# angeladai/sgnn

Hardware: AMD Instinct MI355X
Metric: TSDF blocks/sec fwd+bwd (64^3@5% occ, bs32) (higher is better)
Workload: dtype f32

## Files before the change

sgnn_amd/csrc/bn.hip:

```cpp
#include "common.h"

#define BN_MAX_BLOCKS 2048
#define BN_FLUSH 2
#ifndef BN_U
#define BN_U 2
#endif
#define BN_FUSE_BLOCKS 4096
#define BN_FUSE_MAXC 64

struct BnGeom {
  int vec;
  int cq;
  int rpb;
};

static BnGeom bn_geom(int c) {
  BnGeom g;
  g.vec = (c % 4 == 0) ? 4 : 1;
  g.cq = c / g.vec;
  g.rpb = 256 / g.cq;
  if (g.rpb < 1) g.rpb = 1;
  return g;
}

// ... 6 lines not shown
  return g;
}

static int bn_blocks(int64_t n, const BnGeom &g) {
  int64_t b = (n + (int64_t)g.rpb * BN_FLUSH - 1) / ((int64_t)g.rpb * BN_FLUSH);
  if (b < 1) b = 1;
  if (b > BN_MAX_BLOCKS) b = BN_MAX_BLOCKS;
  return (int)b;
}

SGNN_EXPORT int64_t sgnn_bn_ws_bytes(int64_t n, int c) {
  (void)n;
  return (int64_t)BN_MAX_BLOCKS * 2 * c * (int64_t)sizeof(double) + 4 * (int64_t)c * sizeof(float) + 256;
}

template <int VEC>
__device__ __forceinline__ void load_vec(const float *p, float (&v)[VEC]) {
  if constexpr (VEC == 4) {
    const float4 t = *reinterpret_cast<const float4 *>(p);
    v[0] = t.x; v[1] = t.y; v[2] = t.z; v[3] = t.w;
  } else {
    v[0] = *p;
  }
}
template <int VEC>
__device__ __forceinline__ void store_vec(float *p, const float (&v)[VEC]) {
  if constexpr (VEC == 4) {
    *reinterpret_cast<float4 *>(p) = make_float4(v[0], v[1], v[2], v[3]);
  } else {
    *p = v[0];
  }
}

template <int VEC, int MODE, bool LIN = false>
__global__ __launch_bounds__(256) void k_bn_partial(const float *__restrict__ x, int64_t ldx,
                                                   const float *__restrict__ dy, int64_t ld_dy, int64_t n, int c,
                                                   int cq, int rpb, const float *__restrict__ mean,
                                                   const float *__restrict__ invstd,
                                                   const float *__restrict__ gamma,
                                                   const float *__restrict__ beta, float leak,
                                                   double *__restrict__ partial, const int64_t *n_dev, BnLin lin) {
  extern __shared__ double sh[];
  const int tid = threadIdx.x;
  unsigned nblk = gridDim.x;
  if (n_dev) {
    n = sgnn_dyn_n(n, n_dev);
    int64_t b = (n + (int64_t)rpb * BN_FLUSH - 1) / ((int64_t)rpb * BN_FLUSH);
    if (b < 1) b = 1;
    if (b > BN_MAX_BLOCKS) b = BN_MAX_BLOCKS;
    if (b < (int64_t)nblk) nblk = (unsigned)b;
    if (blockIdx.x >= nblk) {
      for (int o = tid; o < 2 * c; o += 256) partial[(size_t)blockIdx.x * 2 * c + o] = 0.0;
      return;
    }
  }
  const int col = tid % cq, rloc = tid / cq;
  const bool active = rloc < rpb;
  double sa[VEC], sb[VEC];
#pragma unroll
  for (int v = 0; v < VEC; ++v) sa[v] = sb[v] = 0.0;
  float m_[VEC], is_[VEC], g_[VEC], b_[VEC];
  float lw[2][VEC];
  if constexpr (LIN) {
#pragma unroll
    for (int o = 0; o < 2; ++o)
#pragma unroll
      for (int v = 0; v < VEC; ++v) lw[o][v] = (active && o < lin.nout) ? lin.w[o][col * VEC + v] : 0.f;
  }
  if (MODE == 1 && active) {
#pragma unroll
    for (int v = 0; v < VEC; ++v) {
      m_[v] = mean[col * VEC + v];
      is_[v] = invstd[col * VEC + v];
      g_[v] = gamma ? gamma[col * VEC + v] : 1.f;
      b_[v] = beta ? beta[col * VEC + v] : 0.f;
    }
  }
  if (active) {
    const int64_t step = (int64_t)nblk * rpb;
    int64_t row = (int64_t)blockIdx.x * rpb + rloc;
    while (row < n) {
      float fa[VEC], fb[VEC];
#pragma unroll
      for (int v = 0; v < VEC; ++v) fa[v] = fb[v] = 0.f;
      float xv[BN_FLUSH][VEC], dv[BN_FLUSH][VEC];
      bool keep[BN_FLUSH];
#pragma unroll
      for (int it = 0; it < BN_FLUSH; ++it) {
        const int64_t rr = row + it * step;
        keep[it] = rr < n;
        const int64_t rc = rr < n ? rr : row;
        load_vec<VEC>(x + rc * ldx + col * VEC, xv[it]);
        if constexpr (LIN) {
#pragma unroll
          for (int v = 0; v < VEC; ++v) dv[it][v] = 0.f;
#pragma unroll
          for (int o = 0; o < 2; ++o)
            if (o < lin.nout) {
              const float gv = lin.g[rc * lin.ldg + o];
#pragma unroll
              for (int v = 0; v < VEC; ++v) dv[it][v] = fmaf(gv, lw[o][v], dv[it][v]);
            }
        } else if (MODE == 1) {
          load_vec<VEC>(dy + rc * ld_dy + col * VEC, dv[it]);
        }
      }
#pragma unroll
      for (int it = 0; it < BN_FLUSH; ++it) {
        if (MODE == 0) {
#pragma unroll
          for (int v = 0; v < VEC; ++v) {
            const float xm = keep[it] ? xv[it][v] : 0.f;
            fa[v] += xm;
            fb[v] = fmaf(xm, xm, fb[v]);
          }
        } else {
#pragma unroll
          for (int v = 0; v < VEC; ++v) {
            const float xh = (xv[it][v] - m_[v]) * is_[v];
            const float yv = fmaf(xh, g_[v], b_[v]);
            const float dz = keep[it] ? (yv > 0.f ? dv[it][v] : dv[it][v] * leak) : 0.f;
            fa[v] += dz;
            fb[v] = fmaf(dz, xh, fb[v]);
          }
        }
      }
      row += (int64_t)BN_FLUSH * step;
#pragma unroll
      for (int v = 0; v < VEC; ++v) {
        sa[v] += (double)fa[v];
        sb[v] += (double)fb[v];
      }
    }
  }
  double *mine = sh + ((size_t)rloc * cq + col) * 2 * VEC;
// ... 422 lines not shown
                               float leak, float *save_mean, float *save_invstd, float *y, int64_t ldy,
                               const double *pre_partial, int64_t pre_nblk, void *ws, int64_t ws_bytes,
                               sgnn_stream_t stream) {
  return sgnn_bn_fwd_impl(x, ldx, n, c, gamma, beta, running_mean, running_var, eps, momentum, training, leak,
                          save_mean, save_invstd, y, ldy, pre_partial, pre_nblk, ws, ws_bytes, stream);
}

SGNN_EXPORT int sgnn_bn_bwd(const float *x, const float *dy, int64_t n, int c, const float *gamma,
                            const float *beta, const float *save_mean, const float *save_invstd, int training,
                            float leak, float *dx, float *dgamma, float *dbeta, void *ws, int64_t ws_bytes,
                            sgnn_stream_t stream) {
  return sgnn_bn_bwd_impl(x, c, dy, c, n, c, gamma, beta, save_mean, save_invstd, training, leak, nullptr, c, dx, c,
                          dgamma, dbeta, nullptr, 0, ws, ws_bytes, stream);
}

SGNN_EXPORT int sgnn_bn_bwd_add(const float *x, const float *dy, int64_t n, int c, const float *gamma,
                                const float *beta, const float *save_mean, const float *save_invstd, int training,
                                float leak, const float *addend, float *dx, float *dgamma, float *dbeta, void *ws,
                                int64_t ws_bytes, sgnn_stream_t stream) {
  return sgnn_bn_bwd_impl(x, c, dy, c, n, c, gamma, beta, save_mean, save_invstd, training, leak, addend, c, dx, c,
                          dgamma, dbeta, nullptr, 0, ws, ws_bytes, stream);
}

SGNN_EXPORT int sgnn_bn_bwd_ex(const float *x, int64_t ldx, const float *dy, int64_t ld_dy, int64_t n, int c,
                               const float *gamma, const float *beta, const float *save_mean,
                               const float *save_invstd, int training, float leak, const float *addend,
                               int64_t ld_add, float *dx, int64_t ld_dx, float *dgamma, float *dbeta,
                               const double *pre_partial, int64_t pre_nblk, void *ws, int64_t ws_bytes,
                               sgnn_stream_t stream) {
  return sgnn_bn_bwd_impl(x, ldx, dy, ld_dy, n, c, gamma, beta, save_mean, save_invstd, training, leak, addend, ld_add,
                          dx, ld_dx, dgamma, dbeta, pre_partial, pre_nblk, ws, ws_bytes, stream);
}

int sgnn_bn_bwd_impl(const float *x, int64_t ldx, const float *dy, int64_t ld_dy, int64_t n, int c, const float *gamma,
                     const float *beta, const float *save_mean, const float *save_invstd, int training, float leak,
                     const float *addend, int64_t ld_add, float *dx, int64_t ld_dx, float *dgamma, float *dbeta,
                     const double *pre_partial, int64_t pre_nblk, void *ws, int64_t ws_bytes, sgnn_stream_t stream,
                     const int64_t *n_dev, const BnLin *lin) {
  hipStream_t s = (hipStream_t)stream;
  SGNN_CHECK_ARG(n >= 0 && c >= 1 && (c % 4 == 0 ? c <= 1024 : c <= 256) && save_mean && save_invstd);
  SGNN_CHECK_ARG(!lin || (lin->g && lin->nout >= 1 && lin->nout <= 2 && lin->w[0] && (lin->nout < 2 || lin->w[1]) && !pre_partial));
  if (n == 0) {
    if (dgamma) SGNN_HIP_TRY(hipMemsetAsync(dgamma, 0, c * sizeof(float), s));
    if (dbeta) SGNN_HIP_TRY(hipMemsetAsync(dbeta, 0, c * sizeof(float), s));
    return SGNN_OK;
  }
  SGNN_CHECK_ARG(x && (dy || lin) && dx);
  if (ldx <= 0) ldx = c;
  if (ld_dy <= 0) ld_dy = c;
  if (ld_dx <= 0) ld_dx = c;
  if (ld_add <= 0) ld_add = c;
  SGNN_CHECK_ARG(ldx >= c && ld_dy >= c && ld_dx >= c && ld_add >= c);
  if (!ws || ws_bytes < sgnn_bn_ws_bytes(n, c)) {
    sgnn_set_error("sgnn_bn_bwd: workspace too small");
    return SGNN_ENOWS;
  }
  BnGeom g = bn_geom(c);
  if (g.vec == 4 && (ldx % 4 || ld_dy % 4 || ld_dx % 4 || ld_add % 4 || ((uintptr_t)x & 15) || ((uintptr_t)dy & 15) ||
                     ((uintptr_t)dx & 15) || ((uintptr_t)addend & 15)))
    g = bn_geom_scalar(c);
  if (g.cq > 256) {
    sgnn_set_error("sgnn_bn_bwd: %d channels need 16-byte aligned rows (row strides multiples of 4 floats)", c);
    return SGNN_EINVAL;
  }
  const double *partial = pre_partial;
  int64_t nblk = pre_nblk;
  float *coef = (float *)((char *)ws + (size_t)BN_MAX_BLOCKS * 2 * c * sizeof(double));
  if (!partial) {
    nblk = bn_blocks(n, g);
    const size_t shbytes = (size_t)g.rpb * g.cq * 2 * g.vec * sizeof(double);
    if (lin && g.vec == 4)
      SGNN_LAUNCH((k_bn_partial<4, 1, true>), dim3((unsigned)nblk), dim3(256), shbytes, s, x, ldx, dy, ld_dy, n, c, g.cq,
                         g.rpb, save_mean, save_invstd, gamma, beta, leak, (double *)ws, n_dev, *lin);
    else if (lin)
// ... 30 lines not shown
```

sgnn_amd/csrc/common.h:

```cpp
#pragma once
#include <hip/hip_runtime.h>
#include <stdint.h>
#include <stdio.h>
#include "../../include/sgnn_hip.h"

#define SGNN_EXPORT extern "C" __attribute__((visibility("default")))

extern "C" int sgnn_stamp(const char *label, sgnn_stream_t stream);
extern sgnn_tune g_tune;

void sgnn_set_error(const char *fmt, ...);
int sgnn_prof_begin_launch(int kind, int64_t n_out, int cin, int cout, int K, int flags, hipStream_t s);
void sgnn_prof_end_launch(int slot, hipStream_t s);

__device__ __forceinline__ float sgnn_bn_act(float x, float mean, float invstd, float gamma, float beta, float leak) {
  const float xh = (x - mean) * invstd;
  const float t = fmaf(xh, gamma, beta);
  return t > 0.f ? t : t * leak;
}

struct ConvEpi {
  int64_t ldx, ldy, ld_add;
  const float *addend;
  int stats;
  double *partial;
  const float *bn_x;
  int64_t ld_bnx;
  const float *mean, *invstd, *gamma, *beta;
  float leak;
  const int64_t *n_dev;
};

int sgnn_conv_fwd_impl(const float *x, int64_t n_in, int cin, const float *w, int K, const int32_t *table, int64_t ld,
                       int64_t n_out, int cout, float *y, int flags, int in_shift, const int32_t *kmap,
                       const int32_t *kadd, int in_mul, int groups, int table_rows, const ConvEpi *epi,
                       sgnn_stream_t stream);
int64_t sgnn_conv_grid_blocks(int64_t n_out, int cin, int cout, int K);
struct BnLin {
  const float *g;
  int64_t ldg;
  const float *w[2];
  int nout;
};
int sgnn_bn_fwd_impl(const float *x, int64_t ldx, int64_t n, int c, const float *gamma, const float *beta,
                     float *running_mean, float *running_var, float eps, float momentum, int training, float leak,
                     float *save_mean, float *save_invstd, float *y, int64_t ldy, const double *pre_partial,
                     int64_t pre_nblk, void *ws, int64_t ws_bytes, sgnn_stream_t stream, const int64_t *n_dev = nullptr);
int sgnn_bn_bwd_impl(const float *x, int64_t ldx, const float *dy, int64_t ld_dy, int64_t n, int c, const float *gamma,
                     const float *beta, const float *save_mean, const float *save_invstd, int training, float leak,
                     const float *addend, int64_t ld_add, float *dx, int64_t ld_dx, float *dgamma, float *dbeta,
                     const double *pre_partial, int64_t pre_nblk, void *ws, int64_t ws_bytes, sgnn_stream_t stream,
                     const int64_t *n_dev = nullptr, const struct BnLin *lin = nullptr);
bool sgnn_conv_epi_supported(int cin, int cout);
bool dw_shape_ok(int cin, int cout);
#define DW_BATCH_MAX 28
struct DwDesc {
  const float *partial;
  float *dw;
  int64_t nblk, elems;
  int blk0;
};
struct DwBatch {
  DwDesc d[DW_BATCH_MAX];
  int n;
};
extern DwBatch *sgnn_dw_batch;
int sgnn_dw_batch_flush(DwBatch *b, hipStream_t s);
int sgnn_gather_rows_ld(const float *src, int64_t ld_src, int c, const int32_t *idx, int64_t m, float *dst,
                        int64_t ld_dst, sgnn_stream_t stream, const int64_t *n_dev = nullptr);
int sgnn_gather_sum_ld(const float *src, int64_t ld_src, int c, const int32_t *table, int64_t ld, int K, int64_t n_out,
                       float *dst, int64_t ld_dst, sgnn_stream_t stream, const int64_t *n_dev = nullptr);
int sgnn_add_ld(const float *a, int64_t lda, const float *b, int64_t ldb, int64_t n, int c, float *y, int64_t ldy,
                sgnn_stream_t stream, const int64_t *n_dev = nullptr);
int sgnn_fill32(void *p, uint32_t pattern, int64_t words, hipStream_t s);
int sgnn_fill32_multi(void *const *p, const int64_t *words, int nregions, uint32_t pattern, hipStream_t s);
int sgnn_copy_words(void *dst, const void *src, int64_t words, hipStream_t s);
int sgnn_sum_groups_dn(const float *src, int c, int64_t n, int rep, float *dst, sgnn_stream_t stream, const int64_t *n_dev);
int sgnn_concat_rows_dn(const float *a, int ca, const int32_t *ia, const float *b, int cb, const int32_t *ib, int64_t m,
                        float *dst, sgnn_stream_t stream, const int64_t *n_dev);
int sgnn_concat_rows_bwd_dn(const float *ddst, int ca, const int32_t *ia, int cb, const int32_t *ib, int64_t m, float *da,
                            int64_t na, float *db, int64_t nb, sgnn_stream_t stream, const int64_t *n_dev);
int sgnn_concat3_rows_dn(const float *a, int ca, const int32_t *ia, const float *b, int cb, const int32_t *ib,
                         const float *c, int cc, const int32_t *ic, int64_t m, float *dst, sgnn_stream_t stream,
                         const int64_t *n_dev);
int sgnn_concat3_rows_bwd_dn(const float *ddst, int ca, const int32_t *ia, int cb, const int32_t *ib, int cc,
                             const int32_t *ic, int64_t m, float *da, int64_t na, float *db, int64_t nb, float *dc,
                             int64_t nc, sgnn_stream_t stream, const int64_t *n_dev);
int sgnn_conv_bwd_weight_impl(const float *x, int64_t n_in, int cin, int64_t ldx, const float *dy, int cout, int64_t ld_dy,
                              const int32_t *table, int64_t ld, int K, int64_t n_out, float *dw, int in_shift,
                              const int32_t *kmap, const int32_t *kadd, int in_mul, int groups, int table_rows, void *ws,
                              int64_t ws_bytes, sgnn_stream_t stream, const int64_t *n_dev = nullptr);
int sgnn_expand_maps(const int32_t **S, const int32_t **ST, const int32_t **PAR);
int sgnn_linear_fwd_rows(const float *x, int64_t n, int cin, const float *const *w, const float *const *b, int cout,
                         float *y, sgnn_stream_t stream, const int64_t *n_dev = nullptr);
int sgnn_linear_bwd_rows(const float *x, const float *dy, int64_t n, int cin, const float *const *w, int cout,
                         float *dx, float *const *dw, float *const *db, void *ws, int64_t ws_bytes,
                         sgnn_stream_t stream, const int64_t *n_dev = nullptr, const float *addend = nullptr,
                         int64_t ld_add = 0);

extern long long sgnn_launch_counter;
#define SGNN_LAUNCH(...)           \
  do {                             \
    ++sgnn_launch_counter;         \
    hipLaunchKernelGGL(__VA_ARGS__); \
  } while (0)

#define SGNN_CHECK_ARG(cond)                                                    \
  do {                                                                          \
    if (!(cond)) {                                                              \
      sgnn_set_error("%s: invalid argument: %s", __func__, #cond);              \
      return SGNN_EINVAL;                                                       \
    }                                                                           \
  } while (0)

#define SGNN_CHECK_LAUNCH()                                                     \
  do {                                                                          \
    hipError_t e_ = hipGetLastError();                                          \
    if (e_ != hipSuccess) {                                                     \
      sgnn_set_error("%s: HIP error: %s", __func__, hipGetErrorString(e_));     \
      return SGNN_EHIP;                                                         \
    }                                                                           \
  } while (0)

#define SGNN_HIP_TRY(expr)                                                      \
  do {                                                                          \
    hipError_t e_ = (expr);                                                     \
    if (e_ != hipSuccess) {                                                     \
      sgnn_set_error("%s: %s failed: %s", __func__, #expr, hipGetErrorString(e_)); \
      return SGNN_EHIP;                                                         \
    }                                                                           \
  } while (0)
// ... 68 lines not shown
```

sgnn_amd/csrc/linear.hip:

```cpp
#include "common.h"

#define LIN_MAX_OUT 4
#define LIN_MAX_BLOCKS 512

template <int CIN, int VEC>
__device__ __forceinline__ void load_row(const float *__restrict__ p, float (&v)[CIN]) {
  if constexpr (VEC == 4) {
#pragma unroll
    for (int t = 0; t < CIN / 4; ++t) {
      const float4 q = reinterpret_cast<const float4 *>(p)[t];
      v[4 * t] = q.x; v[4 * t + 1] = q.y; v[4 * t + 2] = q.z; v[4 * t + 3] = q.w;
    }
  } else {
#pragma unroll
    for (int t = 0; t < CIN; ++t) v[t] = p[t];
  }
}

struct LinW {
  const float *w[LIN_MAX_OUT];
  const float *b[LIN_MAX_OUT];
};
struct LinG {
  float *dw[LIN_MAX_OUT];
  float *db[LIN_MAX_OUT];
};

template <int CIN, int COUT>
__global__ __launch_bounds__(256) void k_linear_fwd(const float *__restrict__ x, int64_t n, LinW p,
                                                   float *__restrict__ y, const int64_t *n_dev) {
  __shared__ float ws[COUT * CIN + COUT];
  n = sgnn_dyn_n(n, n_dev);
  for (int e = threadIdx.x; e < COUT * CIN; e += 256) ws[e] = p.w[e / CIN][e % CIN];
  if (threadIdx.x < COUT) ws[COUT * CIN + threadIdx.x] = p.b[threadIdx.x] ? p.b[threadIdx.x][0] : 0.f;
  __syncthreads();
  const int64_t stride = (int64_t)gridDim.x * 256;
  for (int64_t r = (int64_t)blockIdx.x * 256 + threadIdx.x; r < n; r += stride) {
    float v[CIN];
    load_row<CIN, (CIN % 4 == 0) ? 4 : 1>(x + r * CIN, v);
#pragma unroll
    for (int o = 0; o < COUT; ++o) {
      float acc = ws[COUT * CIN + o];
#pragma unroll
      for (int c = 0; c < CIN; ++c) acc = fmaf(v[c], ws[o * CIN + c], acc);
      y[r * COUT + o] = acc;
    }
  }
}

template <int CIN, int COUT>
__global__ __launch_bounds__(256) void k_linear_bwd(const float *__restrict__ x, const float *__restrict__ dy,
                                                   int64_t n, LinW p, float *dx, double *__restrict__ partial,
                                                   const int64_t *n_dev, const float *addend, int64_t ld_add) {
  constexpr int NV = COUT * CIN + COUT;
  n = sgnn_dyn_n(n, n_dev);
  __shared__ float ws[COUT * CIN];
  __shared__ float red[4][NV];
  for (int e = threadIdx.x; e < COUT * CIN; e += 256) ws[e] = p.w[e / CIN][e % CIN];
  __syncthreads();
  float acc[NV];
#pragma unroll
  for (int e = 0; e < NV; ++e) acc[e] = 0.f;
  const int64_t stride = (int64_t)gridDim.x * 256;
  for (int64_t r = (int64_t)blockIdx.x * 256 + threadIdx.x; r < n; r += stride) {
    float v[CIN], g[COUT];
    load_row<CIN, (CIN % 4 == 0) ? 4 : 1>(x + r * CIN, v);
#pragma unroll
    for (int o = 0; o < COUT; ++o) g[o] = dy[r * COUT + o];
#pragma unroll
    for (int o = 0; o < COUT; ++o) {
#pragma unroll
      for (int c = 0; c < CIN; ++c) acc[o * CIN + c] = fmaf(g[o], v[c], acc[o * CIN + c]);
      acc[COUT * CIN + o] += g[o];
    }
    if (dx) {
      float d[CIN];
#pragma unroll
      for (int c = 0; c < CIN; ++c) {
        float t = 0.f;
#pragma unroll
        for (int o = 0; o < COUT; ++o) t = fmaf(g[o], ws[o * CIN + c], t);
        d[c] = t;
      }
      if (addend) {
        float a[CIN];
        load_row<CIN, (CIN % 4 == 0) ? 4 : 1>(addend + r * ld_add, a);
#pragma unroll
        for (int c = 0; c < CIN; ++c) d[c] += a[c];
      }
      if constexpr (CIN % 4 == 0) {
#pragma unroll
        for (int t = 0; t < CIN / 4; ++t)
          reinterpret_cast<float4 *>(dx + r * CIN)[t] = make_float4(d[4 * t], d[4 * t + 1], d[4 * t + 2], d[4 * t + 3]);
      } else {
#pragma unroll
        for (int c = 0; c < CIN; ++c) dx[r * CIN + c] = d[c];
      }
    }
  }
  const int lane = threadIdx.x & 63, wave = threadIdx.x >> 6;
#pragma unroll
  for (int e = 0; e < NV; ++e) {
    float t = acc[e];
#pragma unroll
    for (int d = 32; d > 0; d >>= 1) t += __shfl_xor(t, d);
    if (lane == 0) red[wave][e] = t;
  }
  __syncthreads();
  for (int e = threadIdx.x; e < NV; e += 256)
    partial[(size_t)blockIdx.x * NV + e] = (double)red[0][e] + (double)red[1][e] + (double)red[2][e] + (double)red[3][e];
}

__global__ __launch_bounds__(256) void k_linear_finalize(const double *__restrict__ partial, int nblk, int nv,
                                                        int ncw, int cin, LinG g) {
  __shared__ double sh[256];
  const int e = blockIdx.x;
  double a = 0.0;
  for (int b = threadIdx.x; b < nblk; b += 256) a += partial[(size_t)b * nv + e];
  sh[threadIdx.x] = a;
  __syncthreads();
  for (int d = 128; d > 0; d >>= 1) {
    if (threadIdx.x < d) sh[threadIdx.x] += sh[threadIdx.x + d];
    __syncthreads();
  }
  if (threadIdx.x == 0) {
    if (e < ncw) {
      if (g.dw[e / cin]) g.dw[e / cin][e % cin] = (float)sh[0];
    } else if (g.db[e - ncw]) {
      g.db[e - ncw][0] = (float)sh[0];
    }
  }
}

static int lin_blocks(int64_t n) {
  int64_t b = (n + 255) / 256;
  if (b < 1) b = 1;
  if (b > LIN_MAX_BLOCKS) b = LIN_MAX_BLOCKS;
  return (int)b;
}

SGNN_EXPORT int64_t sgnn_linear_ws_bytes(int64_t n, int cin, int cout) {
// ... 24 lines not shown
    SGNN_CHECK_ARG(w[o]);
    p.w[o] = w[o];
    p.b[o] = b ? b[o] : nullptr;
  }
  hipStream_t s = (hipStream_t)stream;
  const int grid = sgnn_grid_for(n, 256, 2048);
  bool done = false;
#define X(CI, CO)                                                                                   \
  if (!done && cin == CI && cout == CO) {                                                           \
    SGNN_LAUNCH((k_linear_fwd<CI, CO>), dim3(grid), dim3(256), 0, s, x, n, p, y, n_dev);     \
    done = true;                                                                                    \
  }
  LIN_CASES(X)
#undef X
  if (!done) {
    sgnn_set_error("sgnn_linear_fwd: unsupported head shape %d -> %d", cin, cout);
    return SGNN_EINVAL;
  }
  SGNN_CHECK_LAUNCH();
  return SGNN_OK;
}

SGNN_EXPORT int sgnn_linear_fwd(const float *x, int64_t n, int cin, const float *w, const float *bias, int cout,
                                float *y, sgnn_stream_t stream) {
  SGNN_CHECK_ARG(cout >= 1 && cout <= LIN_MAX_OUT && cin >= 1);
  const float *wr[LIN_MAX_OUT] = {}, *br[LIN_MAX_OUT] = {};
  for (int o = 0; o < cout; ++o) {
    wr[o] = w ? w + (size_t)o * cin : nullptr;
    br[o] = bias ? bias + o : nullptr;
  }
  return sgnn_linear_fwd_rows(x, n, cin, wr, br, cout, y, stream);
}

int sgnn_linear_bwd_rows(const float *x, const float *dy, int64_t n, int cin, const float *const *w, int cout,
                         float *dx, float *const *dw, float *const *db, void *ws, int64_t ws_bytes,
                         sgnn_stream_t stream, const int64_t *n_dev, const float *addend, int64_t ld_add) {
  hipStream_t s = (hipStream_t)stream;
  SGNN_CHECK_ARG(n >= 0 && cin >= 1 && cout >= 1 && cout <= LIN_MAX_OUT && w);
  SGNN_CHECK_ARG(!addend || (dx && ld_add >= cin && (cin % 4 != 0 || (ld_add % 4 == 0 && ((uintptr_t)addend & 15) == 0))));
  if (!lin_shape_ok(cin, cout)) {
    sgnn_set_error("sgnn_linear_bwd: unsupported head shape %d -> %d", cin, cout);
    return SGNN_EINVAL;
  }
  if (n == 0) {
    for (int o = 0; o < cout; ++o) {
      if (dw && dw[o]) SGNN_HIP_TRY(hipMemsetAsync(dw[o], 0, (size_t)cin * sizeof(float), s));
      if (db && db[o]) SGNN_HIP_TRY(hipMemsetAsync(db[o], 0, sizeof(float), s));
    }
    return SGNN_OK;
  }
  SGNN_CHECK_ARG(x && dy);
  if (!ws || ws_bytes < sgnn_linear_ws_bytes(n, cin, cout)) {
    sgnn_set_error("sgnn_linear_bwd: workspace too small");
    return SGNN_ENOWS;
  }
  LinW p{};
  LinG g{};
  for (int o = 0; o < cout; ++o) {
    SGNN_CHECK_ARG(w[o]);
    p.w[o] = w[o];
    g.dw[o] = dw ? dw[o] : nullptr;
    g.db[o] = db ? db[o] : nullptr;
  }
  const int nblk = lin_blocks(n);
  const int nv = cin * cout + cout;
  bool done = false;
#define X(CI, CO)                                                                                          \
  if (!done && cin == CI && cout == CO) {                                                                  \
    SGNN_LAUNCH((k_linear_bwd<CI, CO>), dim3(nblk), dim3(256), 0, s, x, dy, n, p, dx, (double *)ws, n_dev, addend, ld_add); \
    done = true;                                                                                           \
  }
  LIN_CASES(X)
#undef X
  if (!done) {
    sgnn_set_error("sgnn_linear_bwd: unsupported head shape %d -> %d", cin, cout);
    return SGNN_EINVAL;
  }
  SGNN_LAUNCH(k_linear_finalize, dim3(nv), dim3(256), 0, s, (const double *)ws, nblk, nv, cin * cout, cin, g);
  SGNN_CHECK_LAUNCH();
  return SGNN_OK;
}

SGNN_EXPORT int sgnn_linear_bwd(const float *x, const float *dy, int64_t n, int cin, const float *w, int cout,
                                float *dx, float *dw, float *dbias, void *ws, int64_t ws_bytes,
                                sgnn_stream_t stream) {
  SGNN_CHECK_ARG(cout >= 1 && cout <= LIN_MAX_OUT && cin >= 1 && w);
  const float *wr[LIN_MAX_OUT] = {};
  float *dwr[LIN_MAX_OUT] = {}, *dbr[LIN_MAX_OUT] = {};
  for (int o = 0; o < cout; ++o) {
    wr[o] = w + (size_t)o * cin;
    dwr[o] = dw ? dw + (size_t)o * cin : nullptr;
    dbr[o] = dbias ? dbias + o : nullptr;
  }
  return sgnn_linear_bwd_rows(x, dy, n, cin, wr, cout, dx, dwr, dbr, ws, ws_bytes, stream);
}
```

sgnn_amd/csrc/prog.hip:

```cpp
#include <mutex>
#include <vector>
#include "common.h"

enum {
  OP_CONV_SUBM = 0, OP_CONV_DOWN = 1, OP_UNPOOL = 2, OP_BN = 3, OP_ADD = 4, OP_JOIN = 5,
  OP_CONCAT_IN = 6,
  OP_EXPAND = 7,
  OP_LINEAR = 8
};
#define OPW 12
#define EXPAND_DX_SPLIT 4

extern "C" int sgnn_expand_weights(const float *w, int cin, int cout, float *wc, sgnn_stream_t stream);
extern "C" int sgnn_expand_weights_bwd(const float *dwc, int cin, int cout, float *dw, sgnn_stream_t stream);
int64_t sgnn_bf16_wfrag_bytes(int cin, int cout, int K, int groups);
int sgnn_bf16_conv_prepare(const float *w, int cin, int cout, int K, int groups, void *wf, sgnn_stream_t stream);
int sgnn_bf16_conv_run(const void *x, int64_t n_in, int cin, int64_t ldx, const float *w, const void *wf, int K,
                       const int32_t *table, int64_t ld, int64_t n_out, int cout, void *y, int64_t ldy,
                       const void *addend, int64_t ld_add, const int32_t *kmap, int groups, int table_rows,
                       const int64_t *n_dev, sgnn_stream_t stream);
int sgnn_bf16_conv_expand_impl(const void *x, int64_t n, int cin, int64_t ldx, const float *w, const int32_t *nbr,
                               int64_t ld, int cout, void *y, int64_t ldy, const int64_t *n_dev, void *ws,
                               sgnn_stream_t stream);
int sgnn_bf16_linear_rows(const void *x, int64_t ldx, int64_t n, int cin, const float *const *w, const float *const *b,
// ... 316 lines not shown
  const int32_t *o = v.ops + OPW * i;
  int64_t w = 0;
  if (o[0] == OP_CONV_SUBM) w = sgnn_conv_bwd_weight_ws_bytes(v.lev_n[o[5]], 27, o[6], o[7]);
  if (o[0] == OP_CONV_DOWN) w = sgnn_conv_bwd_weight_ws_bytes(v.lev_n[o[5] + 1], 8, o[6], o[7]);
  if (o[0] == OP_EXPAND)
    w = ((sgnn_conv_bwd_weight_ws_bytes(v.lev_n[o[5]], 64, o[6], o[7]) + 255) & ~int64_t(255)) + expand_dwc_bytes(o[6], o[7]);
  return (w + 255) & ~int64_t(255);
}

int64_t dw_ws_need(const View &v) {
  int64_t need = 0;
  for (int i = 0; i < v.nops; ++i) need += dw_slice(v, i);
  return need;
}

int64_t ws_main(const View &v) {
  int64_t need = 0;
  for (int i = 0; i < v.nops; ++i) {
    const int32_t *o = v.ops + OPW * i;
    int64_t w = 0;
    if (o[0] == OP_BN) w = sgnn_bn_ws_bytes(v.lev_n[o[5]], o[6]);
    if (o[0] == OP_LINEAR) w = sgnn_linear_ws_bytes(v.lev_n[o[5]], o[6], o[7]);
    if (w > need) need = w;
  }
  const int64_t dw = dw_ws_need(v);
  if (dw > need) need = dw;
  return (need + 255) & ~int64_t(255);
}

int64_t ws_stats(const View &v) {
  int64_t need = 0;
  for (int i = 0; i < v.nops; ++i) {
    const int32_t *o = v.ops + OPW * i;
    if (o[0] != OP_CONV_SUBM && o[0] != OP_CONV_DOWN) continue;
    const int64_t rows_f = v.lev_n[o[5]], rows_o = o[0] == OP_CONV_DOWN ? v.lev_n[o[5] + 1] : rows_f;
    const int64_t a = ((rows_o > 0 ? rows_o : 1) + 15) / 16 * 2 * o[7] * (int64_t)sizeof(double);
    const int64_t b = ((rows_f > 0 ? rows_f : 1) + 15) / 16 * 2 * o[6] * (int64_t)sizeof(double);
    if (a > need) need = a;
    if (b > need) need = b;
  }
  return (need + 255) & ~int64_t(255);
}

int64_t ws_need(const View &v) { return ws_main(v) + ws_stats(v); }

struct SideLane {
  hipStream_t stream = nullptr;
  void *ws = nullptr;
  int64_t ws_bytes = 0;
  hipEvent_t fork = nullptr, join = nullptr;
} g_side;
std::mutex g_side_mu;
bool g_defer_join = false;

}

SGNN_EXPORT int sgnn_prog_set_side_stream(sgnn_stream_t stream2, void *ws2, int64_t ws2_bytes) {
  std::lock_guard<std::mutex> hold(g_side_mu);
  if (stream2 && !g_side.fork) {
    SGNN_HIP_TRY(hipEventCreateWithFlags(&g_side.fork, hipEventDisableTiming));
    SGNN_HIP_TRY(hipEventCreateWithFlags(&g_side.join, hipEventDisableTiming));
  }
  g_side.stream = (hipStream_t)stream2;
  g_side.ws = stream2 ? ws2 : nullptr;
  g_side.ws_bytes = stream2 ? ws2_bytes : 0;
  return SGNN_OK;
// ... 369 lines not shown
        alias[b] = -1;
        init[b] = 1;
        return sgnn_add_ld(G(b), LD(b), other, ldo, ROWS(b), CH(b), G(b), LD(b), stream, BCNT(b));
      }
      init[b] = 1;
      return SGNN_OK;
    }
    return sgnn_add_ld(G(b), LD(b), wrote, CH(b), ROWS(b), CH(b), G(b), LD(b), stream, BCNT(b));
  };
  auto wants = [&](int b) { return b >= n_ext || gext[b] != nullptr; };
  std::unique_lock<std::mutex> lane_lock(g_side_mu, std::try_to_lock);
  const bool side = lane_lock.owns_lock() && g_side.stream && g_side.stream != hs && g_side.ws &&
                    g_side.ws_bytes >= dw_ws_need(v);
  bool forked = false;
  auto dw_lane = [&]() -> hipStream_t {
    if (!side) return hs;
    (void)hipEventRecord(g_side.fork, hs);
    (void)hipStreamWaitEvent(g_side.stream, g_side.fork, 0);
    forked = true;
    return g_side.stream;
  };
  char *dw_base = (char *)(side ? g_side.ws : ws);
  int64_t dw_off = 0;
  DwBatch batch{};
  struct BatchGuard {
    explicit BatchGuard(DwBatch *b) { sgnn_dw_batch = b; }
    ~BatchGuard() { sgnn_dw_batch = nullptr; }
  } guard(side ? &batch : nullptr);
  struct PendingExpand { const float *dwc; int cin, cout; float *dw; };
  std::vector<PendingExpand> pending_expand;
  std::vector<const double *> pre(nops, nullptr);
  std::vector<int64_t> pre_nblk(nops, 0);
  double *stats_ws = (double *)((char *)ws + ws_main(v));

  for (int i = nops - 1; i >= 0; --i) {
    const int32_t *o = ops + OPW * i;
    const int type = o[0], in0 = o[1], in1 = o[2], out = o[3], par = o[4], lev = o[5], cin = o[6], cout = o[7];
    const int64_t n = lev_n[lev];
    if (!init[out] && !(type == OP_BN && lazy_lin[out] >= 0)) {
      if (type == OP_CONV_SUBM || type == OP_CONV_DOWN || type == OP_EXPAND)
        PROG_TRY(sgnn_fill32(PG(par), 0u, (int64_t)(type == OP_CONV_DOWN ? 8 : 27) * cin * cout, hs));
      if (type == OP_BN) {
        {
          void *zp[2] = {PG(par), PG(par + 1)};
          const int64_t zw[2] = {cin, cin};
          PROG_TRY(sgnn_fill32_multi(zp, zw, 2, 0u, hs));
        }
      }
      if (type == OP_LINEAR)
        for (int q = 0; q < cout; ++q) {
          void *zp[2] = {PG(par + 2 * q), PG(par + 2 * q + 1)};
          const int64_t zw[2] = {cin, 1};
          PROG_TRY(sgnn_fill32_multi(zp, zw, 2, 0u, hs));
        }
      continue;
    }
    const float *dy = GR(out);
    const int64_t ld_dy = GRLD(out);
    switch (type) {
      case OP_CONV_SUBM:
      case OP_CONV_DOWN: {
        const bool down = type == OP_CONV_DOWN;
        const int K = down ? 8 : 27;
        const int64_t n_dy = down ? lev_n[lev + 1] : n;
        const int32_t *tab_f = (const int32_t *)(down ? lev_children[lev] : lev_nbr[lev]);
        const int64_t ld_f = down ? lev_ld[lev + 1] : lev_ld[lev];
// ... 119 lines not shown
      case OP_CONCAT_IN: {
        const int src[3] = {in0, in1, o[8]};
        float *d[3] = {nullptr, nullptr, nullptr};
        for (int q = 0; q < 3; ++q)
          if (src[q] >= 0 && wants(src[q])) {
            if (init[src[q]]) {
              sgnn_set_error("sgnn_prog_backward: a CONCAT_IN source already carries a gradient (unsupported)");
              return SGNN_EINVAL;
            }
            d[q] = G(src[q]);
            init[src[q]] = 1;
          }
        SGNN_CHECK_ARG(ld_dy == CH(out));
        PROG_TRY(sgnn_concat3_rows_bwd_dn(dy, CH(in0), I(o[9]), CH(in1), I(o[10]), CH(o[8]), I(o[11]), n, d[0],
                                          in0 >= 0 ? ROWS(in0) : 0, d[1], in1 >= 0 ? ROWS(in1) : 0, d[2],
                                          o[8] >= 0 ? ROWS(o[8]) : 0, stream, CNT(lev)));
        break;
      }
      case OP_EXPAND: {
        const int32_t *S, *ST, *PAR;
        PROG_TRY(sgnn_expand_maps(&S, &ST, &PAR));
        const float *wc = arena + L.aux_off[i];
        const int32_t *nbr = (const int32_t *)lev_nbr[lev];
        float *dwc = side ? (float *)(dw_base + dw_off + dw_slice(v, i) - expand_dwc_bytes(cin, cout)) : garena + L.bextra;
        float *part = garena + L.bextra + round64(64 * (int64_t)cin * cout);
        const hipStream_t lane = dw_lane();
        SGNN_CHECK_ARG(ld_dy == cout && LD(in0) == cin);
        if (wants(in0) && n > 0) {
          const int Gs = EXPAND_DX_SPLIT;
          ConvEpi xepi{};
          xepi.n_dev = CNT(lev);
          PROG_TRY(sgnn_conv_fwd_impl(dy, 8 * n, cout, wc, 64 / Gs, nbr, lev_ld[lev], n, cin, part, SGNN_CONV_TRANSPOSE_W,
                                      0, ST, PAR, 8, Gs, 27, &xepi, stream));
          float *t = target(in0, 0);
          PROG_TRY(sgnn_sum_groups_dn(part, cin, n, Gs, t, stream, CNT(lev)));
          PROG_TRY(commit(in0, t));
        }
        {
          PROG_TRY(sgnn_conv_bwd_weight_impl(X(in0), n, cin, cin, dy, cout, cout, nbr, lev_ld[lev], 8, n, dwc, 0, S, nullptr, 1,
                                             8, 27, dw_base + dw_off, dw_slice(v, i), (sgnn_stream_t)lane, CNT(lev)));
        }
        dw_off += dw_slice(v, i);
        pending_expand.push_back(PendingExpand{dwc, cin, cout, PG(par)});
        break;
      }
      case OP_LINEAR: {
        const float *w[4] = {};
        float *dw[4] = {}, *db[4] = {};
        for (int q = 0; q < cout; ++q) {
          w[q] = P(par + 2 * q);
          dw[q] = PG(par + 2 * q);
          db[q] = PG(par + 2 * q + 1);
        }
        SGNN_CHECK_ARG(ld_dy == cout && LD(in0) == cin);
        if (PL.lin_bn[i] >= 0 && wants(in0) && !init[in0] && n > 0 && !pre[PL.lin_bn[i]]) {
          PROG_TRY(sgnn_linear_bwd_rows(X(in0), dy, n, cin, w, cout, nullptr, dw, db, ws, ws_bytes, stream, CNT(lev)));
          lazy_lin[in0] = i;
          break;
        }
        const float *have = (g_fuse && g_lin_add && wants(in0) && init[in0] && n > 0) ? GR(in0) : nullptr;
        const int64_t have_ld = have ? GRLD(in0) : 0;
        if (have && have_ld % 4 == 0 && ((uintptr_t)have & 15) == 0 && !viewed[in0]) {
          PROG_TRY(sgnn_linear_bwd_rows(X(in0), dy, n, cin, w, cout, G(in0), dw, db, ws, ws_bytes, stream, CNT(lev), have,
                                        have_ld));
          alias[in0] = -1;
          init[in0] = 1;
          break;
        }
        float *t = wants(in0) ? target(in0, 0) : nullptr;
        PROG_TRY(sgnn_linear_bwd_rows(X(in0), dy, n, cin, w, cout, t, dw, db, ws, ws_bytes, stream, CNT(lev)));
        if (t) PROG_TRY(commit(in0, t));
        break;
      }
      default:
        sgnn_set_error("sgnn_prog_backward: unknown op %d", type);
        return SGNN_EINVAL;
    }
  }
  for (int b = 0; b < n_ext; ++b) {
    if (!gext[b] || L.buf_floats[b] == 0) continue;
    if (init[b] == 2)
      PROG_TRY(sgnn_copy_words(G(b), GR(b), L.buf_floats[b], hs));
    else if (init[b] == 0)
      PROG_TRY(sgnn_fill32(G(b), 0u, L.buf_floats[b], hs));
  }
  {
    const hipStream_t lane = side ? g_side.stream : hs;
    PROG_TRY(sgnn_dw_batch_flush(&batch, lane));
    for (const PendingExpand &pe : pending_expand)
      PROG_TRY(sgnn_expand_weights_bwd(pe.dwc, pe.cin, pe.cout, pe.dw, (sgnn_stream_t)lane));
  }
  if (forked && !g_defer_join) {
    SGNN_HIP_TRY(hipEventRecord(g_side.join, g_side.stream));
    SGNN_HIP_TRY(hipStreamWaitEvent(hs, g_side.join, 0));
  }
  return SGNN_OK;
}
```

Before: 5589.

## Fuse BN backward statistics into linear backward and expand group-sum kernels

Computes the batch-norm backward partial reductions (sum of dz and dz*xhat) inside the producer kernels, namely the linear-head backward and the expand group-sum, when a BN op directly precedes them. The partials are handed to the following BN backward as precomputed input. This removes a separate read pass over x and dy. The cost is extra registers and shared memory in the linear kernel, a widened stats workspace, and more complex bookkeeping in the program's backward pass.

```diff
diff --git a/sgnn_amd/csrc/bn.hip b/sgnn_amd/csrc/bn.hip
--- a/sgnn_amd/csrc/bn.hip
+++ b/sgnn_amd/csrc/bn.hip
@@ -62,14 +62,22 @@
   }
 }
 
-template <int VEC, int MODE, bool LIN = false>
+struct BnSumG {
+  const float *src;
+  int rep;
+  float *dst;
+  int64_t ld_dst;
+};
+
+template <int VEC, int MODE, bool LIN = false, bool SUMG = false>
 __global__ __launch_bounds__(256) void k_bn_partial(const float *__restrict__ x, int64_t ldx,
                                                    const float *__restrict__ dy, int64_t ld_dy, int64_t n, int c,
                                                    int cq, int rpb, const float *__restrict__ mean,
                                                    const float *__restrict__ invstd,
                                                    const float *__restrict__ gamma,
                                                    const float *__restrict__ beta, float leak,
-                                                   double *__restrict__ partial, const int64_t *n_dev, BnLin lin) {
+                                                   double *__restrict__ partial, const int64_t *n_dev, BnLin lin,
+                                                   BnSumG sg = BnSumG{}) {
   extern __shared__ double sh[];
   const int tid = threadIdx.x;
   unsigned nblk = gridDim.x;
@@ -131,6 +139,27 @@
 #pragma unroll
               for (int v = 0; v < VEC; ++v) dv[it][v] = fmaf(gv, lw[o][v], dv[it][v]);
             }
+        } else if constexpr (SUMG) {
+          const float *p = sg.src + rc * sg.rep * c + col * VEC;
+#pragma unroll
+          for (int v = 0; v < VEC; ++v) dv[it][v] = 0.f;
+          int t = 0;
+          for (; t + 4 <= sg.rep; t += 4) {
+            float s4[4][VEC];
+#pragma unroll
+            for (int u = 0; u < 4; ++u) load_vec<VEC>(p + (int64_t)(t + u) * c, s4[u]);
+#pragma unroll
+            for (int u = 0; u < 4; ++u)
+#pragma unroll
+              for (int v = 0; v < VEC; ++v) dv[it][v] += s4[u][v];
+          }
+          for (; t < sg.rep; ++t) {
+            float s1[VEC];
+            load_vec<VEC>(p + (int64_t)t * c, s1);
+#pragma unroll
+            for (int v = 0; v < VEC; ++v) dv[it][v] += s1[v];
+          }
+          if (keep[it]) store_vec<VEC>(sg.dst + rc * sg.ld_dst + col * VEC, dv[it]);
         } else if (MODE == 1) {
           load_vec<VEC>(dy + rc * ld_dy + col * VEC, dv[it]);
         }
@@ -619,6 +648,31 @@
                           dx, ld_dx, dgamma, dbeta, pre_partial, pre_nblk, ws, ws_bytes, stream);
 }
 
+int64_t sgnn_bn_stats_blocks_max(void) { return BN_MAX_BLOCKS; }
+
+int sgnn_bn_bwd_stats_sum_groups(const float *src, int rep, int64_t n, int c, float *dst, int64_t ld_dst, const BnStatsIn &bn,
+                                 int64_t *nblk, sgnn_stream_t stream, const int64_t *n_dev) {
+  hipStream_t s = (hipStream_t)stream;
+  SGNN_CHECK_ARG(n > 0 && rep >= 1 && c >= 1 && (c % 4 == 0 ? c <= 1024 : c <= 256) && src && dst && nblk && ld_dst >= c);
+  SGNN_CHECK_ARG(bn.x && bn.mean && bn.invstd && bn.partial && bn.ldx >= c);
+  BnGeom g = bn_geom(c);
+  if (g.vec == 4 && (bn.ldx % 4 || ld_dst % 4 || ((uintptr_t)bn.x & 15) || ((uintptr_t)dst & 15) || ((uintptr_t)src & 15)))
+    g = bn_geom_scalar(c);
+  SGNN_CHECK_ARG(g.cq <= 256);
+  const int64_t nb = bn_blocks(n, g);
+  const size_t shbytes = (size_t)g.rpb * g.cq * 2 * g.vec * sizeof(double);
+  const BnSumG sg{src, rep, dst, ld_dst};
+  if (g.vec == 4)
+    SGNN_LAUNCH((k_bn_partial<4, 1, false, true>), dim3((unsigned)nb), dim3(256), shbytes, s, bn.x, bn.ldx, nullptr, 0, n, c,
+                g.cq, g.rpb, bn.mean, bn.invstd, bn.gamma, bn.beta, bn.leak, bn.partial, n_dev, BnLin{}, sg);
+  else
+    SGNN_LAUNCH((k_bn_partial<1, 1, false, true>), dim3((unsigned)nb), dim3(256), shbytes, s, bn.x, bn.ldx, nullptr, 0, n, c,
+                g.cq, g.rpb, bn.mean, bn.invstd, bn.gamma, bn.beta, bn.leak, bn.partial, n_dev, BnLin{}, sg);
+  SGNN_CHECK_LAUNCH();
+  *nblk = nb;
+  return SGNN_OK;
+}
+
 int sgnn_bn_bwd_impl(const float *x, int64_t ldx, const float *dy, int64_t ld_dy, int64_t n, int c, const float *gamma,
                      const float *beta, const float *save_mean, const float *save_invstd, int training, float leak,
                      const float *addend, int64_t ld_add, float *dx, int64_t ld_dx, float *dgamma, float *dbeta,
@@ -626,7 +680,7 @@
                      const int64_t *n_dev, const BnLin *lin) {
   hipStream_t s = (hipStream_t)stream;
   SGNN_CHECK_ARG(n >= 0 && c >= 1 && (c % 4 == 0 ? c <= 1024 : c <= 256) && save_mean && save_invstd);
-  SGNN_CHECK_ARG(!lin || (lin->g && lin->nout >= 1 && lin->nout <= 2 && lin->w[0] && (lin->nout < 2 || lin->w[1]) && !pre_partial));
+  SGNN_CHECK_ARG(!lin || (lin->g && lin->nout >= 1 && lin->nout <= 2 && lin->w[0] && (lin->nout < 2 || lin->w[1])));
   if (n == 0) {
     if (dgamma) SGNN_HIP_TRY(hipMemsetAsync(dgamma, 0, c * sizeof(float), s));
     if (dbeta) SGNN_HIP_TRY(hipMemsetAsync(dbeta, 0, c * sizeof(float), s));
diff --git a/sgnn_amd/csrc/common.h b/sgnn_amd/csrc/common.h
--- a/sgnn_amd/csrc/common.h
+++ b/sgnn_amd/csrc/common.h
@@ -42,6 +42,13 @@
   const float *w[2];
   int nout;
 };
+struct BnStatsIn {
+  const float *x;
+  int64_t ldx;
+  const float *mean, *invstd, *gamma, *beta;
+  float leak;
+  double *partial;
+};
 int sgnn_bn_fwd_impl(const float *x, int64_t ldx, int64_t n, int c, const float *gamma, const float *beta,
                      float *running_mean, float *running_var, float eps, float momentum, int training, float leak,
                      float *save_mean, float *save_invstd, float *y, int64_t ldy, const double *pre_partial,
@@ -51,6 +58,9 @@
                      const float *addend, int64_t ld_add, float *dx, int64_t ld_dx, float *dgamma, float *dbeta,
                      const double *pre_partial, int64_t pre_nblk, void *ws, int64_t ws_bytes, sgnn_stream_t stream,
                      const int64_t *n_dev = nullptr, const struct BnLin *lin = nullptr);
+int sgnn_bn_bwd_stats_sum_groups(const float *src, int rep, int64_t n, int c, float *dst, int64_t ld_dst, const BnStatsIn &bn,
+                                 int64_t *nblk, sgnn_stream_t stream, const int64_t *n_dev);
+int64_t sgnn_bn_stats_blocks_max(void);
 bool sgnn_conv_epi_supported(int cin, int cout);
 bool dw_shape_ok(int cin, int cout);
 #define DW_BATCH_MAX 28
@@ -96,7 +106,9 @@
 int sgnn_linear_bwd_rows(const float *x, const float *dy, int64_t n, int cin, const float *const *w, int cout,
                          float *dx, float *const *dw, float *const *db, void *ws, int64_t ws_bytes,
                          sgnn_stream_t stream, const int64_t *n_dev = nullptr, const float *addend = nullptr,
-                         int64_t ld_add = 0);
+                         int64_t ld_add = 0, const BnStatsIn *bn = nullptr, int64_t *bn_nblk = nullptr);
+bool sgnn_linear_bn_stats_ok(int cin, int cout, const BnStatsIn &bn);
+int64_t sgnn_linear_blocks_max(void);
 
 extern long long sgnn_launch_counter;
 #define SGNN_LAUNCH(...)           \
diff --git a/sgnn_amd/csrc/linear.hip b/sgnn_amd/csrc/linear.hip
--- a/sgnn_amd/csrc/linear.hip
+++ b/sgnn_amd/csrc/linear.hip
@@ -48,22 +48,72 @@
   }
 }
 
-template <int CIN, int COUT>
+template <int CIN, int COUT, int BNS>
 __global__ __launch_bounds__(256) void k_linear_bwd(const float *__restrict__ x, const float *__restrict__ dy,
                                                    int64_t n, LinW p, float *dx, double *__restrict__ partial,
-                                                   const int64_t *n_dev, const float *addend, int64_t ld_add) {
+                                                   const int64_t *n_dev, const float *addend, int64_t ld_add,
+                                                   BnStatsIn bn) {
   constexpr int NV = COUT * CIN + COUT;
   n = sgnn_dyn_n(n, n_dev);
   __shared__ float ws[COUT * CIN];
   __shared__ float red[4][NV];
+  __shared__ float4 bnc[BNS ? CIN : 1];
+  __shared__ double redb[4][BNS ? 2 * CIN : 1];
   for (int e = threadIdx.x; e < COUT * CIN; e += 256) ws[e] = p.w[e / CIN][e % CIN];
+  if constexpr (BNS != 0)
+    for (int e = threadIdx.x; e < CIN; e += 256)
+      bnc[e] = make_float4(bn.mean[e], bn.invstd[e], bn.gamma ? bn.gamma[e] : 1.f, bn.beta ? bn.beta[e] : 0.f);
   __syncthreads();
   float acc[NV];
 #pragma unroll
   for (int e = 0; e < NV; ++e) acc[e] = 0.f;
+  float sb[BNS ? 2 * CIN : 1];
+#pragma unroll
+  for (int e = 0; e < (BNS ? 2 * CIN : 1); ++e) sb[e] = 0.f;
   const int64_t stride = (int64_t)gridDim.x * 256;
   for (int64_t r = (int64_t)blockIdx.x * 256 + threadIdx.x; r < n; r += stride) {
-    float v[CIN], g[COUT];
+    float g[COUT];
+    if constexpr (BNS != 0) {
+      constexpr int DV = (CIN % 4 == 0) ? 4 : 1;
+      float xb[CIN], ad[BNS == 2 ? CIN : 1];
+      load_row<CIN, DV>(bn.x + r * bn.ldx, xb);
+      if constexpr (BNS == 2) load_row<CIN, DV>(addend + r * ld_add, ad);
+#pragma unroll
+      for (int o = 0; o < COUT; ++o) g[o] = dy[r * COUT + o];
+#pragma unroll
+      for (int c0 = 0; c0 < CIN; c0 += DV) {
+        float d[DV];
+#pragma unroll
+        for (int j = 0; j < DV; ++j) {
+          const int c = c0 + j;
+          int cl = c;
+          asm volatile("" : "+v"(cl));
+          const float4 k = bnc[cl];
+          const float xh = (xb[c] - k.x) * k.y;
+          const float t = fmaf(xh, k.z, k.w);
+          const float a = t > 0.f ? t : t * bn.leak;
+          float dd = 0.f;
+#pragma unroll
+          for (int o = 0; o < COUT; ++o) {
+            acc[o * CIN + c] = fmaf(g[o], a, acc[o * CIN + c]);
+            dd = fmaf(g[o], ws[o * CIN + cl], dd);
+          }
+          if constexpr (BNS == 2) dd += ad[c];
+          d[j] = dd;
+          const float dz = t > 0.f ? dd : dd * bn.leak;
+          sb[c] += dz;
+          sb[CIN + c] = fmaf(dz, xh, sb[CIN + c]);
+        }
+        if (dx) {
+          if constexpr (DV == 4) *reinterpret_cast<float4 *>(dx + r * CIN + c0) = make_float4(d[0], d[1], d[2], d[3]);
+          else dx[r * CIN + c0] = d[0];
+        }
+      }
+#pragma unroll
+      for (int o = 0; o < COUT; ++o) acc[COUT * CIN + o] += g[o];
+      continue;
+    }
+    float v[CIN];
     load_row<CIN, (CIN % 4 == 0) ? 4 : 1>(x + r * CIN, v);
 #pragma unroll
     for (int o = 0; o < COUT; ++o) g[o] = dy[r * COUT + o];
@@ -106,7 +156,20 @@
     for (int d = 32; d > 0; d >>= 1) t += __shfl_xor(t, d);
     if (lane == 0) red[wave][e] = t;
   }
+  if constexpr (BNS != 0) {
+#pragma unroll
+    for (int e = 0; e < 2 * CIN; ++e) {
+      double t = (double)sb[e];
+#pragma unroll
+      for (int d = 32; d > 0; d >>= 1) t += __shfl_xor(t, d);
+      if (lane == 0) redb[wave][e] = t;
+      if ((e & 7) == 7) __builtin_amdgcn_sched_barrier(0);
+    }
+  }
   __syncthreads();
+  if constexpr (BNS != 0)
+    for (int e = threadIdx.x; e < 2 * CIN; e += 256)
+      bn.partial[(size_t)blockIdx.x * 2 * CIN + e] = ((redb[0][e] + redb[1][e]) + redb[2][e]) + redb[3][e];
   for (int e = threadIdx.x; e < NV; e += 256)
     partial[(size_t)blockIdx.x * NV + e] = (double)red[0][e] + (double)red[1][e] + (double)red[2][e] + (double)red[3][e];
 }
@@ -197,12 +260,23 @@
   return sgnn_linear_fwd_rows(x, n, cin, wr, br, cout, y, stream);
 }
 
+int64_t sgnn_linear_blocks_max(void) { return LIN_MAX_BLOCKS; }
+
+static constexpr bool lin_bns_fits(int cin, int cout) { return cin * cout + cout + 2 * cin <= 160; }
+
+bool sgnn_linear_bn_stats_ok(int cin, int cout, const BnStatsIn &bn) {
+  return lin_bns_fits(cin, cout) && bn.x && bn.mean && bn.invstd && bn.partial && bn.ldx >= cin &&
+         (cin % 4 != 0 || (bn.ldx % 4 == 0 && ((uintptr_t)bn.x & 15) == 0));
+}
+
 int sgnn_linear_bwd_rows(const float *x, const float *dy, int64_t n, int cin, const float *const *w, int cout,
                          float *dx, float *const *dw, float *const *db, void *ws, int64_t ws_bytes,
-                         sgnn_stream_t stream, const int64_t *n_dev, const float *addend, int64_t ld_add) {
+                         sgnn_stream_t stream, const int64_t *n_dev, const float *addend, int64_t ld_add,
+                         const BnStatsIn *bn, int64_t *bn_nblk) {
   hipStream_t s = (hipStream_t)stream;
   SGNN_CHECK_ARG(n >= 0 && cin >= 1 && cout >= 1 && cout <= LIN_MAX_OUT && w);
   SGNN_CHECK_ARG(!addend || (dx && ld_add >= cin && (cin % 4 != 0 || (ld_add % 4 == 0 && ((uintptr_t)addend & 15) == 0))));
+  SGNN_CHECK_ARG(!bn || (n > 0 && bn_nblk && sgnn_linear_bn_stats_ok(cin, cout, *bn)));
   if (!lin_shape_ok(cin, cout)) {
     sgnn_set_error("sgnn_linear_bwd: unsupported head shape %d -> %d", cin, cout);
     return SGNN_EINVAL;
@@ -230,13 +304,25 @@
   const int nblk = lin_blocks(n);
   const int nv = cin * cout + cout;
   bool done = false;
+  const BnStatsIn bs = bn ? *bn : BnStatsIn{};
 #define X(CI, CO)                                                                                          \
   if (!done && cin == CI && cout == CO) {                                                                  \
-    SGNN_LAUNCH((k_linear_bwd<CI, CO>), dim3(nblk), dim3(256), 0, s, x, dy, n, p, dx, (double *)ws, n_dev, addend, ld_add); \
+    if constexpr (lin_bns_fits(CI, CO)) {                                                                  \
+      if (bn && addend)                                                                                    \
+        SGNN_LAUNCH((k_linear_bwd<CI, CO, 2>), dim3(nblk), dim3(256), 0, s, x, dy, n, p, dx, (double *)ws, n_dev, addend, \
+                    ld_add, bs);                                                                           \
+      else if (bn)                                                                                         \
+        SGNN_LAUNCH((k_linear_bwd<CI, CO, 1>), dim3(nblk), dim3(256), 0, s, x, dy, n, p, dx, (double *)ws, n_dev, addend, \
+                    ld_add, bs);                                                                           \
+    }                                                                                                      \
+    if (!bn)                                                                                               \
+      SGNN_LAUNCH((k_linear_bwd<CI, CO, 0>), dim3(nblk), dim3(256), 0, s, x, dy, n, p, dx, (double *)ws, n_dev, addend, \
+                  ld_add, bs);                                                                             \
     done = true;                                                                                           \
   }
   LIN_CASES(X)
 #undef X
+  if (bn) *bn_nblk = nblk;
   if (!done) {
     sgnn_set_error("sgnn_linear_bwd: unsupported head shape %d -> %d", cin, cout);
     return SGNN_EINVAL;
diff --git a/sgnn_amd/csrc/prog.hip b/sgnn_amd/csrc/prog.hip
--- a/sgnn_amd/csrc/prog.hip
+++ b/sgnn_amd/csrc/prog.hip
@@ -372,6 +372,11 @@
   int64_t need = 0;
   for (int i = 0; i < v.nops; ++i) {
     const int32_t *o = v.ops + OPW * i;
+    if (o[0] == OP_LINEAR || o[0] == OP_EXPAND) {
+      const int64_t blocks = o[0] == OP_LINEAR ? sgnn_linear_blocks_max() : sgnn_bn_stats_blocks_max();
+      const int64_t a = blocks * 2 * o[6] * (int64_t)sizeof(double);
+      if (a > need) need = a;
+    }
     if (o[0] != OP_CONV_SUBM && o[0] != OP_CONV_DOWN) continue;
     const int64_t rows_f = v.lev_n[o[5]], rows_o = o[0] == OP_CONV_DOWN ? v.lev_n[o[5] + 1] : rows_f;
     const int64_t a = ((rows_o > 0 ? rows_o : 1) + 15) / 16 * 2 * o[7] * (int64_t)sizeof(double);
@@ -807,6 +812,14 @@
   std::vector<const double *> pre(nops, nullptr);
   std::vector<int64_t> pre_nblk(nops, 0);
   double *stats_ws = (double *)((char *)ws + ws_main(v));
+  auto bn_before = [&](int i, int b, int c, int lev, BnStatsIn &bs) -> bool {
+    if (!g_fuse || i <= 0) return false;
+    const int32_t *bo = ops + OPW * (i - 1);
+    if (bo[0] != OP_BN || bo[3] != b || bo[6] != c || bo[5] != lev) return false;
+    const float *save = arena + L.aux_off[i - 1];
+    bs = BnStatsIn{X(bo[1]), LD(bo[1]), save, save + c, P(bo[4]), P(bo[4] + 1), opf[4 * (i - 1) + 2], stats_ws};
+    return true;
+  };
 
   for (int i = nops - 1; i >= 0; --i) {
     const int32_t *o = ops + OPW * i;
@@ -992,9 +1005,16 @@
           xepi.n_dev = CNT(lev);
           PROG_TRY(sgnn_conv_fwd_impl(dy, 8 * n, cout, wc, 64 / Gs, nbr, lev_ld[lev], n, cin, part, SGNN_CONV_TRANSPOSE_W,
                                       0, ST, PAR, 8, Gs, 27, &xepi, stream));
-          float *t = target(in0, 0);
-          PROG_TRY(sgnn_sum_groups_dn(part, cin, n, Gs, t, stream, CNT(lev)));
-          PROG_TRY(commit(in0, t));
+          BnStatsIn bs{};
+          if (!init[in0] && bn_before(i, in0, cin, lev, bs)) {
+            PROG_TRY(sgnn_bn_bwd_stats_sum_groups(part, Gs, n, cin, G(in0), LD(in0), bs, &pre_nblk[i - 1], stream, CNT(lev)));
+            pre[i - 1] = stats_ws;
+            init[in0] = 1;
+          } else {
+            float *t = target(in0, 0);
+            PROG_TRY(sgnn_sum_groups_dn(part, cin, n, Gs, t, stream, CNT(lev)));
+            PROG_TRY(commit(in0, t));
+          }
         }
         {
           PROG_TRY(sgnn_conv_bwd_weight_impl(X(in0), n, cin, cin, dy, cout, cout, nbr, lev_ld[lev], 8, n, dwc, 0, S, nullptr, 1,
@@ -1013,8 +1033,16 @@
           db[q] = PG(par + 2 * q + 1);
         }
         SGNN_CHECK_ARG(ld_dy == cout && LD(in0) == cin);
+        BnStatsIn bs{};
+        const bool bn_in_front = n > 0 && wants(in0) && bn_before(i, in0, cin, lev, bs) && sgnn_linear_bn_stats_ok(cin, cout, bs);
+        auto handed = [&](bool on) {
+          if (on) pre[i - 1] = stats_ws;
+        };
         if (PL.lin_bn[i] >= 0 && wants(in0) && !init[in0] && n > 0 && !pre[PL.lin_bn[i]]) {
-          PROG_TRY(sgnn_linear_bwd_rows(X(in0), dy, n, cin, w, cout, nullptr, dw, db, ws, ws_bytes, stream, CNT(lev)));
+          const bool st = bn_in_front && PL.lin_bn[i] == i - 1;
+          PROG_TRY(sgnn_linear_bwd_rows(X(in0), dy, n, cin, w, cout, nullptr, dw, db, ws, ws_bytes, stream, CNT(lev), nullptr, 0,
+                                        st ? &bs : nullptr, st ? &pre_nblk[i - 1] : nullptr));
+          handed(st);
           lazy_lin[in0] = i;
           break;
         }
@@ -1022,13 +1050,17 @@
         const int64_t have_ld = have ? GRLD(in0) : 0;
         if (have && have_ld % 4 == 0 && ((uintptr_t)have & 15) == 0 && !viewed[in0]) {
           PROG_TRY(sgnn_linear_bwd_rows(X(in0), dy, n, cin, w, cout, G(in0), dw, db, ws, ws_bytes, stream, CNT(lev), have,
-                                        have_ld));
+                                        have_ld, bn_in_front ? &bs : nullptr, bn_in_front ? &pre_nblk[i - 1] : nullptr));
+          handed(bn_in_front);
           alias[in0] = -1;
           init[in0] = 1;
           break;
         }
         float *t = wants(in0) ? target(in0, 0) : nullptr;
-        PROG_TRY(sgnn_linear_bwd_rows(X(in0), dy, n, cin, w, cout, t, dw, db, ws, ws_bytes, stream, CNT(lev)));
+        const bool st = bn_in_front && !init[in0];
+        PROG_TRY(sgnn_linear_bwd_rows(X(in0), dy, n, cin, w, cout, t, dw, db, ws, ws_bytes, stream, CNT(lev), nullptr, 0,
+                                      st ? &bs : nullptr, st ? &pre_nblk[i - 1] : nullptr));
+        handed(st);
         if (t) PROG_TRY(commit(in0, t));
         break;
       }
```

Result: no change. 5588 (-0.0%).
